# HazyResearch/hyena-dna

Measured on NVIDIA H100. Metric: nucleotides/sec through HyenaOperator fwd+bwd at L=1M d=256, higher is better.
Workload: dtype f32

## Files before the change

hyena-dna_b200/csrc/k_proj.cu:

```cuda
#include <cstdint>
#include <cstring>

#include "../../include/hyena_b200.h"
#include "launch.h"
#include "proj_gemm.cuh"

namespace hy {

static_assert(FN_GELU_TANH == HYENA_B200_GELU_TANH && FN_GELU_ERF == HYENA_B200_GELU_ERF, "activation codes of the C ABI");

size_t proj_wimg_bytes(int N, int K) {
  const int NT = 128;
  return pg::wimg_floats(N, K, NT) * sizeof(float);
}

typedef CUresult (*EncodeTiledFn)(CUtensorMap*, CUtensorMapDataType, cuuint32_t, void*, const cuuint64_t*, const cuuint64_t*,
                                  const cuuint32_t*, const cuuint32_t*, CUtensorMapInterleave, CUtensorMapSwizzle,
                                  CUtensorMapL2promotion, CUtensorMapFloatOOBfill);
static EncodeTiledFn encode_tiled() {
  static EncodeTiledFn fn = [] {
    void* p = nullptr;
    cudaDriverEntryPointQueryResult q;
    if (cudaGetDriverEntryPoint("cuTensorMapEncodeTiled", &p, cudaEnableDefault, &q) != cudaSuccess ||
        q != cudaDriverEntryPointSuccess)
      p = nullptr;
    return reinterpret_cast<EncodeTiledFn>(p);
  }();
  return fn;
}

static bool make_tmap(CUtensorMap* m, const float* base, unsigned long long rows, unsigned long long cols, unsigned box_cols,
                      unsigned box_rows, bool swizzle128) {
  EncodeTiledFn f = encode_tiled();
  if (!f) return false;
  cuuint64_t dims[2] = {cols, rows};
  cuuint64_t strides[1] = {cols * sizeof(float)};
  cuuint32_t box[2] = {box_cols, box_rows};
  cuuint32_t estr[2] = {1, 1};
  return f(m, CU_TENSOR_MAP_DATA_TYPE_FLOAT32, 2, const_cast<float*>(base), dims, strides, box, estr,
           CU_TENSOR_MAP_INTERLEAVE_NONE, swizzle128 ? CU_TENSOR_MAP_SWIZZLE_128B : CU_TENSOR_MAP_SWIZZLE_NONE,
           CU_TENSOR_MAP_L2_PROMOTION_L2_256B, CU_TENSOR_MAP_FLOAT_OOB_FILL_NONE) == CUDA_SUCCESS;
}

static bool make_tmap3(CUtensorMap* m, const float* base, unsigned long long d0, unsigned long long d1, unsigned long long d2,
                       unsigned b0, unsigned b1) {
  EncodeTiledFn f = encode_tiled();
  if (!f) return false;
  cuuint64_t dims[3] = {d0, d1, d2};
  cuuint64_t strides[2] = {d0 * sizeof(float), d0 * d1 * sizeof(float)};
  cuuint32_t box[3] = {b0, b1, 1};
  cuuint32_t estr[3] = {1, 1, 1};
  return f(m, CU_TENSOR_MAP_DATA_TYPE_FLOAT32, 3, const_cast<float*>(base), dims, strides, box, estr,
           CU_TENSOR_MAP_INTERLEAVE_NONE, CU_TENSOR_MAP_SWIZZLE_NONE, CU_TENSOR_MAP_L2_PROMOTION_L2_256B,
           CU_TENSOR_MAP_FLOAT_OOB_FILL_NONE) == CUDA_SUCCESS;
}

template <int NT, int ACT, int OUT, int FN = FN_NONE>
static cudaError_t go(pg::Args a, int sms, cudaStream_t s, int kind = K_PROJ_GEMM) {
  auto kern = pg::proj_gemm_kernel<NT, ACT, OUT, FN>;
  CUtensorMap tmap;
  memset(&tmap, 0, sizeof(tmap));
  if (a.vec) {
    const bool ok = (ACT == pg::ACT_ROW)
        ? make_tmap(&tmap, a.act, (unsigned long long)a.B * a.L, (unsigned long long)a.K, 32, 128, true)
        : make_tmap(&tmap, a.act, (unsigned long long)a.B * a.K, (unsigned long long)a.L, 132, 32, false);
    if (!ok) a.vec = 0;
  }
  const size_t smem = pg::Cfg<NT>::SMEM + (a.fir ? (size_t)a.K * 12 : 0);
  if (smem > 227 * 1024) return cudaErrorInvalidValue;
  cudaError_t e = cudaFuncSetAttribute(kern, cudaFuncAttributeMaxDynamicSharedMemorySize, (int)smem);
  if (e != cudaSuccess) return e;
  const long long ntiles = (long long)a.B * a.mtiles_per_b * a.ntiles_n;
  const int grid = (int)(ntiles < sms ? ntiles : sms);
  prof_begin(kind, s);
  kern<<<grid, pg::kThreads, smem, s>>>(a, tmap);
  prof_end(kind, s);
  return cudaGetLastError();
}

template <int NT>
static cudaError_t by_layout(const pg::Args& a, int act_layout, int out_layout, int sms, cudaStream_t s) {
  if (act_layout == pg::ACT_ROW && out_layout == pg::OUT_CH) return go<NT, pg::ACT_ROW, pg::OUT_CH>(a, sms, s);
  if (act_layout == pg::ACT_ROW && out_layout == pg::OUT_ROW) return go<NT, pg::ACT_ROW, pg::OUT_ROW>(a, sms, s);
  if (act_layout == pg::ACT_CH && out_layout == pg::OUT_CH) return go<NT, pg::ACT_CH, pg::OUT_CH>(a, sms, s);
  if (act_layout == pg::ACT_CH && out_layout == pg::OUT_ROW) return go<NT, pg::ACT_CH, pg::OUT_ROW>(a, sms, s);
  return cudaErrorInvalidValue;
}

cudaError_t launch_proj_gemm(const float* act, int act_layout, const float* W, int ldw, int w_transposed, const float* bias,
                             const float* fir, float* out, int out_layout, int B, int L, int K, int N, int l0, int ln,
                             float* wimg, cudaStream_t s, int fn, const float* aux) {
  const int NT = 128;
  int dev = 0, sms = 132;
  cudaGetDevice(&dev);
  cudaDeviceGetAttribute(&sms, cudaDevAttrMultiProcessorCount, dev);
  const size_t total = pg::wimg_floats(N, K, NT);
  int pblocks = (int)((total + 255) / 256);
  if (pblocks > 4 * sms) pblocks = 4 * sms;
  prof_begin(K_PROJ_PREP, s);
  pg::proj_prep_kernel<<<pblocks, 256, 0, s>>>(W, ldw, w_transposed, N, K, NT, wimg);
  prof_end(K_PROJ_PREP, s);
  cudaError_t e = cudaGetLastError();
  if (e != cudaSuccess) return e;
  pg::Args a;
  a.act = act; a.wimg = wimg; a.out = out; a.bias = bias; a.fir = fir; a.aux = aux;
  a.B = B; a.L = L; a.K = K; a.N = N; a.l0 = l0; a.ln = ln;
  if (act_layout == pg::ACT_ROW) a.vec = (K % 4 == 0);
  else a.vec = (L % 4 == 0) && (l0 % 4 == 0);
  a.kchunks = (K + pg::kKC - 1) / pg::kKC;
  a.ntiles_n = (N + NT - 1) / NT;
  a.mtiles_per_b = (ln + 127) / 128;
  if (fn == FN_NONE) return by_layout<128>(a, act_layout, out_layout, sms, s);
  if (act_layout == pg::ACT_CH && out_layout == pg::OUT_ROW) {
    if (fn == FN_GELU_TANH) return go<128, pg::ACT_CH, pg::OUT_ROW, FN_GELU_TANH>(a, sms, s, K_PROJ_GEMM_GELU);
    if (fn == FN_GELU_ERF) return go<128, pg::ACT_CH, pg::OUT_ROW, FN_GELU_ERF>(a, sms, s, K_PROJ_GEMM_GELU);
  }
  if (act_layout == pg::ACT_ROW && out_layout == pg::OUT_CH) {
    if (fn == FN_GELU_TANH) return go<128, pg::ACT_ROW, pg::OUT_CH, FN_GELU_TANH>(a, sms, s, K_PROJ_GEMM_DGELU);
    if (fn == FN_GELU_ERF) return go<128, pg::ACT_ROW, pg::OUT_CH, FN_GELU_ERF>(a, sms, s, K_PROJ_GEMM_DGELU);
  }
  return cudaErrorInvalidValue;
}


void proj_wgrad_plan(int M, int N, int sms, int* mtiles, int* ntiles, int* splits) {
  *mtiles = (M + 127) / 128;
  *ntiles = (N + 127) / 128;
  int s = sms / (*mtiles * *ntiles);
  *splits = s < 1 ? 1 : s;
}

size_t proj_wgrad_scratch_bytes(int M, int N) {
  int dev = 0, sms = 132, mt, nt, sp;
  cudaGetDevice(&dev);
  cudaDeviceGetAttribute(&sms, cudaDevAttrMultiProcessorCount, dev);
  proj_wgrad_plan(M, N, sms, &mt, &nt, &sp);
  return (size_t)sp * M * N * sizeof(float);
}

cudaError_t launch_proj_wgrad(const float* X, const float* Y, const float* fir, float* dW, int transposed_out, float beta,
                              int B, int L, int M, int N, float* part, cudaStream_t s, int fn) {
  int dev = 0, sms = 132;
  cudaGetDevice(&dev);
  cudaDeviceGetAttribute(&sms, cudaDevAttrMultiProcessorCount, dev);
  wg::Args a;
  a.X = X; a.Y = Y; a.fir = fir; a.part = part; a.zero = 0; a.B = B; a.L = L; a.M = M; a.N = N;
  a.chunks_per_b = (L + 31) / 32;
  proj_wgrad_plan(M, N, sms, &a.mtiles, &a.ntiles, &a.splits);
  const long long total_chunks = (long long)B * a.chunks_per_b;
  if (a.splits > total_chunks) a.splits = (int)total_chunks;
  a.vec = (L % 4 == 0) && (N % 4 == 0) && ((reinterpret_cast<uintptr_t>(X) | reinterpret_cast<uintptr_t>(Y)) & 15u) == 0;
  CUtensorMap tmx, tmy;
  memset(&tmx, 0, sizeof(tmx)); memset(&tmy, 0, sizeof(tmy));
  if (a.vec) {
    const bool ok = make_tmap3(&tmx, X, (unsigned long long)L, (unsigned long long)M, (unsigned long long)B, 36, 128) &&
                    make_tmap3(&tmy, Y, (unsigned long long)N, (unsigned long long)L, (unsigned long long)B, 128, 32);
    if (!ok) a.vec = 0;
  }
  auto kern = fn == FN_GELU_TANH ? wg::wgrad_kernel<FN_GELU_TANH>
            : fn == FN_GELU_ERF  ? wg::wgrad_kernel<FN_GELU_ERF> : wg::wgrad_kernel<FN_NONE>;
  if (fn != FN_NONE && (fir || (fn != FN_GELU_TANH && fn != FN_GELU_ERF))) return cudaErrorInvalidValue;
  const int kind = fn == FN_NONE ? K_PROJ_WGRAD : K_PROJ_WGRAD_GELU;
  cudaError_t e = cudaFuncSetAttribute(kern, cudaFuncAttributeMaxDynamicSharedMemorySize, (int)wg::kSmem);
  if (e != cudaSuccess) return e;
  prof_begin(kind, s);
  kern<<<a.mtiles * a.ntiles * a.splits, wg::kThreads, wg::kSmem, s>>>(a, tmx, tmy);
  prof_end(kind, s);
  e = cudaGetLastError();
  if (e != cudaSuccess) return e;
  const size_t total = (size_t)M * N;
  int blocks = (int)((total + 255) / 256);
  if (blocks > 2 * sms) blocks = 2 * sms;
  prof_begin(kind, s);
  wg::wgrad_reduce_kernel<<<blocks, 256, 0, s>>>(part, dW, a.splits, M, N, transposed_out, beta);
  prof_end(kind, s);
  return cudaGetLastError();
}

}
```

hyena-dna_b200/csrc/proj_gemm.cuh:

```cuda
#pragma once
#include <cuda.h>

#include "common.cuh"
#include "tc_prims.cuh"

namespace hy {

enum ActFn { FN_NONE = 0, FN_GELU_TANH = 1, FN_GELU_ERF = 2 };

template <int FN>
__device__ __forceinline__ float act_fn(float x) {
  static_assert(FN == FN_GELU_TANH || FN == FN_GELU_ERF, "GELU variant");
  if constexpr (FN == FN_GELU_TANH) {
    constexpr float kBeta = (float)(M_SQRT2 * M_2_SQRTPI * 0.5), kKappa = 0.044715f;
    const float inner = kBeta * (x + kKappa * (x * x * x));
    return 0.5f * x * (1.f + tanhf(inner));
  } else {
    return x * 0.5f * (1.f + erff(x * (float)M_SQRT1_2));
  }
}

template <int FN>
__device__ __forceinline__ float act_grad(float x) {
  static_assert(FN == FN_GELU_TANH || FN == FN_GELU_ERF, "GELU variant");
  if constexpr (FN == FN_GELU_TANH) {
    constexpr float kBeta = (float)(M_SQRT2 * M_2_SQRTPI * 0.5), kKappa = 0.044715f;
    const float x_sq = x * x;
    const float th = tanhf(kBeta * (x + kKappa * (x_sq * x)));
    const float left = 0.5f * x, right = 1.f + th;
    const float left_derivative = 0.5f * right;
    const float right_derivative = left * (1.f - th * th) * (kBeta * (1.f + 3.f * kKappa * x_sq));
    return left_derivative + right_derivative;
  } else {
    constexpr float kBeta = (float)(M_2_SQRTPI * M_SQRT1_2 * 0.5);
    const float cdf = 0.5f * (1.f + erff(x * (float)M_SQRT1_2));
    const float pdf = expf(-0.5f * x * x) * kBeta;
    return cdf + x * pdf;
  }
}

namespace pg {

constexpr int kKC = 32;
constexpr int kThreads = 288;
constexpr uint32_t kSBO = 1024, kLBO = 128;
constexpr uint32_t kAPitchCh = 132 * 4;
constexpr uint32_t kAStageBytes = 32 * kAPitchCh;

__host__ __device__ constexpr uint32_t img_off(int n, int k) {
  return (uint32_t)((n >> 3) * 1024 + (k >> 2) * 128 + (n & 7) * 16 + (k & 3) * 4);
}

enum ActLayout { ACT_ROW = 0 , ACT_CH = 1  };
enum OutLayout { OUT_CH = 0 , OUT_ROW = 1  };

struct Args {
  const float* act;
  const float* wimg;
  float* out;
  const float* bias;
  const float* fir;
  int B, L, K, N;
  int l0, ln;
  int kchunks;
  int ntiles_n;
  int mtiles_per_b;
  int vec;
  const float* aux;
};

__global__ void proj_prep_kernel(const float* __restrict__ W, int ldw, int transposed, int N, int K, int NT,
                                 float* __restrict__ img) {
  const int kch = (K + kKC - 1) / kKC, ntn = (N + NT - 1) / NT;
  const size_t total = (size_t)ntn * kch * NT * kKC;
  for (size_t i = (size_t)blockIdx.x * blockDim.x + threadIdx.x; i < total; i += (size_t)gridDim.x * blockDim.x) {
    const int kk = (int)(i % kKC);
    const int nn = (int)((i / kKC) % NT);
    const int kc = (int)((i / ((size_t)kKC * NT)) % kch);
    const int nt = (int)(i / ((size_t)kKC * NT * kch));
    const int n = nt * NT + nn, k = kc * kKC + kk;
    float x = 0.f;
    if (n < N && k < K) x = transposed ? W[(size_t)k * ldw + n] : W[(size_t)n * ldw + k];
    float hi, lo;
    tc::split_tf32(x, hi, lo);
    float* base = img + ((size_t)nt * kch + kc) * 2 * NT * kKC;
    base[img_off(nn, kk) / 4] = hi;
    base[(size_t)NT * kKC + img_off(nn, kk) / 4] = lo;
  }
}

__host__ __device__ constexpr size_t wimg_floats(int N, int K, int NT) {
  return (size_t)((N + NT - 1) / NT) * ((K + kKC - 1) / kKC) * 2 * NT * kKC;
}

constexpr uint32_t kSStageBytes = 17408;
static_assert(kSStageBytes >= 32 * kAPitchCh && kSStageBytes >= 128 * 128 && kSStageBytes % 1024 == 0, "staging slot");

template <int NT> struct Cfg {
  static constexpr int STAGES = 4;
  static constexpr uint32_t STAGE_BYTES = 2u * NT * kKC * 4u;
  static constexpr size_t OFF_A = (size_t)STAGES * STAGE_BYTES;
  static constexpr size_t OFF_BAR = OFF_A + (size_t)STAGES * kSStageBytes;
  static constexpr size_t OFF_FIR = OFF_BAR + 256;
  static constexpr size_t SMEM = OFF_FIR;
  static_assert(NT == 128, "one m64n128 accumulator per consumer warpgroup");
};

template <int NT, int ACT, int OUT, int FN = FN_NONE>
__global__ void __launch_bounds__(kThreads, 1) proj_gemm_kernel(const Args a, const __grid_constant__ CUtensorMap tmap) {
  static_assert(FN == FN_NONE || (ACT == ACT_CH && OUT == OUT_ROW) || (ACT == ACT_ROW && OUT == OUT_CH),
                "the GELU transforms exist for the fc2 forward and input-gradient layouts only");
  using C = Cfg<NT>;
  extern __shared__ __align__(1024) unsigned char smem[];
  uint64_t* bars = reinterpret_cast<uint64_t*>(smem + C::OFF_BAR);
  float* fir_s = reinterpret_cast<float*>(smem + C::OFF_FIR);
  const uint32_t sbase = tc::smem_u32(smem);
  const uint32_t bar0 = tc::smem_u32(bars);
  auto FULL = [&](int s) { return bar0 + 8u * s; };
  auto EMPTY = [&](int s) { return bar0 + 8u * (4 + s); };

  const int tid = threadIdx.x, warp = tid >> 5, lane = tid & 31;
  const bool use_fir = (ACT == ACT_CH) && a.fir != nullptr;
  if (use_fir)
    for (int i = tid; i < 3 * a.K; i += kThreads) fir_s[i] = __ldg(a.fir + i);
  if (tid == 0) {
    for (int s = 0; s < 4; ++s) { tc::mbar_init(FULL(s), 1); tc::mbar_init(EMPTY(s), 8); }
  }
  __syncthreads();

  const int mtiles = a.B * a.mtiles_per_b;
  const int ntiles = mtiles * a.ntiles_n;
  const int lend = a.l0 + a.ln;
  auto tile_pos = [&](int tile, int& b, int& lt, int& nt) {
    const int mt = tile / a.ntiles_n;
    nt = tile - mt * a.ntiles_n;
    b = mt / a.mtiles_per_b;
    lt = a.l0 + (mt - b * a.mtiles_per_b) * 128;
  };

  if (warp == 8) {
    if (lane == 0 && a.vec) tc::tma_prefetch_desc(&tmap);
    uint32_t it = 0;
    for (int tile = blockIdx.x; tile < ntiles; tile += gridDim.x) {
      int b, lt, nt;
      tile_pos(tile, b, lt, nt);
      for (int kc = 0; kc < a.kchunks; ++kc, ++it) {
        const int s = (int)(it & 3u);
        const int k0 = kc * kKC;
        tc::mbar_wait_u(EMPTY(s), ((it >> 2) & 1u) ^ 1u);
        const float* wsrc = a.wimg + ((size_t)nt * a.kchunks + kc) * (C::STAGE_BYTES / 4);
        const uint32_t st_u = sbase + (uint32_t)C::OFF_A + (uint32_t)s * kSStageBytes;
        if (a.vec) {
          if (lane == 0) {
            const uint32_t abytes = (ACT == ACT_ROW) ? 128u * 128u : 32u * kAPitchCh;
            tc::mbar_arrive_expect_tx(FULL(s), C::STAGE_BYTES + abytes);
            tc::bulk_g2s(sbase + s * C::STAGE_BYTES, wsrc, C::STAGE_BYTES, FULL(s));
            if constexpr (ACT == ACT_ROW) tc::tma_load_2d(st_u, &tmap, k0, b * a.L + lt, FULL(s));
            else tc::tma_load_2d(st_u, &tmap, lt, b * a.K + k0, FULL(s));
          }
          continue;
        }
        unsigned char* st = smem + C::OFF_A + (size_t)s * kSStageBytes;
        if constexpr (ACT == ACT_ROW) {
#pragma unroll 1
          for (int i = 0; i < 4; ++i) {
            const int r = lane + 32 * i, l = lt + r;
            const float* src = a.act + ((size_t)b * a.L + (l < lend ? l : 0)) * a.K + k0;
#pragma unroll
            for (int c = 0; c < 8; ++c) {
              float4 v;
              v.x = (l < lend && k0 + 4 * c + 0 < a.K) ? __ldg(src + 4 * c + 0) : 0.f;
              v.y = (l < lend && k0 + 4 * c + 1 < a.K) ? __ldg(src + 4 * c + 1) : 0.f;
              v.z = (l < lend && k0 + 4 * c + 2 < a.K) ? __ldg(src + 4 * c + 2) : 0.f;
              v.w = (l < lend && k0 + 4 * c + 3 < a.K) ? __ldg(src + 4 * c + 3) : 0.f;
              *reinterpret_cast<float4*>(st + r * 128 + ((c ^ (r & 7)) << 4)) = v;
            }
          }
        } else {
          const int j = lane;
          const bool kv = k0 + j < a.K;
          const float* src = a.act + ((size_t)b * a.K + (kv ? k0 + j : 0)) * a.L + lt;
          float* dst = reinterpret_cast<float*>(st + j * kAPitchCh);
          for (int e = 0; e < 132; ++e) dst[e] = (kv && lt + e < a.L) ? __ldg(src + e) : 0.f;
        }
        __syncwarp();
        if (lane == 0) {
          tc::mbar_arrive_expect_tx(FULL(s), C::STAGE_BYTES);
          tc::bulk_g2s(sbase + s * C::STAGE_BYTES, wsrc, C::STAGE_BYTES, FULL(s));
        }
      }
    }
    return;
  }

  const int wg = warp >> 2, g = lane >> 2, t = lane & 3;
  const int r0 = 64 * wg + 16 * (warp & 3) + g;
  uint32_t it = 0;
  for (int tile = blockIdx.x; tile < ntiles; tile += gridDim.x) {
    int b, lt, nt;
    tile_pos(tile, b, lt, nt);
    float sum[64], acc[64];
    for (int kc = 0; kc < a.kchunks; ++kc, ++it) {
      const int s = (int)(it & 3u);
      tc::mbar_wait_u(FULL(s), (it >> 2) & 1u);
      const unsigned char* st = smem + C::OFF_A + (size_t)s * kSStageBytes;
      const int k0 = kc * kKC;
      uint32_t ahi[4][4], alo[4][4];
#pragma unroll
      for (int ks = 0; ks < 4; ++ks) {
#pragma unroll
        for (int q = 0; q < 4; ++q) {
          const int row = r0 + ((q & 1) ? 8 : 0), k = 8 * ks + t + ((q & 2) ? 4 : 0);
          float x;
          if constexpr (ACT == ACT_ROW) {
            x = *reinterpret_cast<const float*>(st + row * 128 + (((k >> 2) ^ (row & 7)) << 4) + (k & 3) * 4);
          } else {
            const float* sp = reinterpret_cast<const float*>(st + k * kAPitchCh) + row;
            if constexpr (FN != FN_NONE) {
              x = act_fn<FN>(sp[0]);
            } else if (!use_fir) {
              x = sp[0];
            } else {
              const float* w = fir_s + 3 * (k0 + k < a.K ? k0 + k : 0);
              x = fmaf(w[2], sp[0], fmaf(w[1], sp[1], w[0] * sp[2]));
            }
          }
          float hh, lw;
          tc::split_tf32(x, hh, lw);
          ahi[ks][q] = __float_as_uint(hh); alo[ks][q] = __float_as_uint(lw);
        }
      }
      const uint32_t bhi = sbase + s * C::STAGE_BYTES, blo = bhi + C::STAGE_BYTES / 2;
      tc::wgmma_fence();
      tc::fence_regs(acc);
#pragma unroll
      for (int ks = 0; ks < 4; ++ks) {
        tc::wgmma_rs_n128(acc, alo[ks], tc::make_desc_ls(bhi + ks * 2 * kLBO, kLBO, kSBO), ks ? 1u : 0u);
        tc::wgmma_rs_n128(acc, ahi[ks], tc::make_desc_ls(blo + ks * 2 * kLBO, kLBO, kSBO), 1u);
      }
#pragma unroll
      for (int ks = 0; ks < 4; ++ks)
        tc::wgmma_rs_n128(acc, ahi[ks], tc::make_desc_ls(bhi + ks * 2 * kLBO, kLBO, kSBO), 1u);
      tc::wgmma_commit();
      tc::wgmma_wait<0>();
      tc::fence_regs(acc);
      __syncwarp();
      if (lane == 0) tc::mbar_arrive(EMPTY(s));
      if (kc == 0) {
#pragma unroll
        for (int i = 0; i < 64; ++i) sum[i] = acc[i];
      } else {
#pragma unroll
        for (int i = 0; i < 64; ++i) sum[i] += acc[i];
      }
    }
#pragma unroll
    for (int h = 0; h < 2; ++h) {
      const int l = lt + r0 + 8 * h;
      if (l >= lend) continue;
      float pre[16];
#pragma unroll
      for (int j = 0; j < 16; ++j) {
        if constexpr (OUT == OUT_CH && FN != FN_NONE) {
          if (j % 8 == 0) {
#pragma unroll
            for (int i = 0; i < 16; ++i) {
              const int n = nt * NT + 8 * (j + (i >> 1)) + 2 * t + (i & 1);
              pre[i] = n < a.N ? __ldg(a.aux + ((size_t)b * a.N + n) * a.L + l) : 0.f;
            }
          }
        }
        const int n = nt * NT + 8 * j + 2 * t;
        float v0 = sum[4 * j + 2 * h], v1 = sum[4 * j + 2 * h + 1];
        if constexpr (OUT == OUT_CH && FN != FN_NONE) {
          float* dst = a.out + ((size_t)b * a.N + n) * a.L + l;
          if (n < a.N) dst[0] = v0 * act_grad<FN>(pre[2 * (j % 8)]);
          if (n + 1 < a.N) dst[a.L] = v1 * act_grad<FN>(pre[2 * (j % 8) + 1]);
        } else if constexpr (OUT == OUT_CH) {
          float* dst = a.out + ((size_t)b * a.N + n) * a.L + l;
          if (n < a.N) dst[0] = v0 + (a.bias ? __ldg(a.bias + n) : 0.f);
          if (n + 1 < a.N) dst[a.L] = v1 + (a.bias ? __ldg(a.bias + n + 1) : 0.f);
        } else {
          float* dst = a.out + ((size_t)b * a.L + l) * a.N + n;
          if (a.bias) {
            if (n < a.N) v0 += __ldg(a.bias + n);
            if (n + 1 < a.N) v1 += __ldg(a.bias + n + 1);
          }
          if (n + 1 < a.N && (a.N & 1) == 0) *reinterpret_cast<float2*>(dst) = make_float2(v0, v1);
          else {
            if (n < a.N) dst[0] = v0;
            if (n + 1 < a.N) dst[1] = v1;
          }
        }
      }
    }
  }
}

}

namespace wg {

constexpr int kThreads = 512;
constexpr int kRegConsumer = 184, kRegConvert = 88, kRegProducer = 56;
static_assert(2 * kRegConsumer + kRegConvert + kRegProducer <= 4 * 128, "register file of one CTA");
constexpr int kSeg = 4;
constexpr int kStg = 4;
constexpr uint32_t kYPitch = 128 * 4;
constexpr uint32_t kYStage = 32 * kYPitch;
constexpr uint32_t kXPitch = 36 * 4;
constexpr uint32_t kXStage = 128 * kXPitch;
constexpr uint32_t kImg = 128 * 32 * 4;
constexpr uint32_t kOffY = 0, kOffX = kOffY + kStg * kYStage;
constexpr uint32_t kOffImg = (kOffX + kStg * kXStage + 1023u) & ~1023u;
constexpr uint32_t kOffBar = kOffImg + 2 * 2 * kImg;
constexpr size_t kSmem = kOffBar + 256;
static_assert(kOffImg % 1024 == 0, "operand images must start on a core-matrix group boundary");
static_assert(kYStage % 128 == 0 && kXStage % 128 == 0, "TMA destinations are 128-byte aligned");
static_assert(kSmem <= 227 * 1024, "shared memory budget");

struct Args {
  const float* X;
  const float* Y;
  const float* fir;
  float* part;
  int B, L, M, N;
  int chunks_per_b;
  int mtiles, ntiles, splits;
  int vec;
  unsigned zero;
};

template <int FN = FN_NONE>
__global__ void __launch_bounds__(kThreads, 1) wgrad_kernel(const Args a, const __grid_constant__ CUtensorMap tmapX,
                                                            const __grid_constant__ CUtensorMap tmapY) {
  extern __shared__ __align__(1024) unsigned char smem[];
  uint64_t* bars = reinterpret_cast<uint64_t*>(smem + kOffBar);
  const uint32_t sbase = tc::smem_u32(smem), bar0 = tc::smem_u32(bars);
  auto B_FULL = [&](int s) { return bar0 + 8u * s; };
  auto B_EMPTY = [&](int s) { return bar0 + 8u * (2 + s); };
  auto S_FULL = [&](int j) { return bar0 + 8u * (4 + j); };
  auto Y_EMPTY = [&](int j) { return bar0 + 8u * (8 + j); };
  auto X_EMPTY = [&](int j) { return bar0 + 8u * (12 + j); };
  const int tid = threadIdx.x, warp = tid >> 5, lane = tid & 31;

  if (tid == 0) {
    for (int s = 0; s < 2; ++s) { tc::mbar_init(B_FULL(s), 128); tc::mbar_init(B_EMPTY(s), 8); }
    for (int j = 0; j < kStg; ++j) { tc::mbar_init(S_FULL(j), 1); tc::mbar_init(Y_EMPTY(j), 256); tc::mbar_init(X_EMPTY(j), 128); }
  }
  __syncthreads();

  const int split = blockIdx.x % a.splits;
  const int tile = blockIdx.x / a.splits;
  const int nt = tile / a.mtiles, mt = tile - nt * a.mtiles;
  const int n0 = nt * 128, m0 = mt * 128;
  const int nrows = min(128, a.N - n0);
  const int mcols = min(128, a.M - m0);
  const long long total_chunks = (long long)a.B * a.chunks_per_b;
  const long long c_begin = total_chunks * split / a.splits, c_end = total_chunks * (split + 1) / a.splits;
  const long long nchunks = c_end - c_begin;

  if (warp < 8) {
    tc::setmaxnreg_inc<kRegConsumer>();
    const int wgi = warp >> 2, g = lane >> 2, t = lane & 3;
    const int nl0 = 64 * wgi + 16 * (warp & 3) + g;
    float acc[64], sum[64], yv[4][4];
#pragma unroll
    for (int i = 0; i < 64; ++i) sum[i] = 0.f;
    auto load_y = [&](long long q) {
      const int ss = (int)(q % kStg);
      tc::mbar_wait_u(S_FULL(ss), (uint32_t)(q / kStg) & 1u);
      const unsigned char* st = smem + kOffY + (size_t)ss * kYStage;
      uint32_t dep = 0;
#pragma unroll
      for (int ks = 0; ks < 4; ++ks) {
#pragma unroll
        for (int e = 0; e < 4; ++e) {
          const int nl = nl0 + ((e & 1) ? 8 : 0), k = 8 * ks + t + ((e & 2) ? 4 : 0);
          yv[ks][e] = *reinterpret_cast<const float*>(st + k * kYPitch + nl * 4);
          dep |= __float_as_uint(yv[ks][e]);
        }
      }
      tc::mbar_arrive_after_loads(Y_EMPTY(ss), dep, a.zero);
    };
    if (nchunks > 0) load_y(0);
    for (long long q = 0; q < nchunks; ++q) {
      uint32_t ahi[4][4], alo[4][4];
#pragma unroll
      for (int ks = 0; ks < 4; ++ks) {
#pragma unroll
        for (int e = 0; e < 4; ++e) {
          float h, lw;
          tc::split_tf32(yv[ks][e], h, lw);
          ahi[ks][e] = __float_as_uint(h); alo[ks][e] = __float_as_uint(lw);
        }
      }
      const uint32_t it = (uint32_t)q;
      const int s = it & 1;
      tc::mbar_wait_u(B_FULL(s), (it >> 1) & 1);
      const uint32_t bhi = sbase + kOffImg + s * 2 * kImg, blo = bhi + kImg;
      const uint32_t cont = (it % kSeg) != 0;
      tc::wgmma_fence();
      tc::fence_regs(acc);
#pragma unroll
      for (int ks = 0; ks < 4; ++ks) {
        tc::wgmma_rs_n128(acc, alo[ks], tc::make_desc_ls(bhi + ks * 2 * pg::kLBO, pg::kLBO, pg::kSBO), (cont | ks) ? 1u : 0u);
        tc::wgmma_rs_n128(acc, ahi[ks], tc::make_desc_ls(blo + ks * 2 * pg::kLBO, pg::kLBO, pg::kSBO), 1u);
      }
#pragma unroll
      for (int ks = 0; ks < 4; ++ks)
        tc::wgmma_rs_n128(acc, ahi[ks], tc::make_desc_ls(bhi + ks * 2 * pg::kLBO, pg::kLBO, pg::kSBO), 1u);
      tc::wgmma_commit();
      if (q + 1 < nchunks) load_y(q + 1);
      tc::wgmma_wait<0>();
      tc::fence_regs(acc);
      tc::fence_frags(ahi);
      tc::fence_frags(alo);
      __syncwarp();
      if (lane == 0) tc::mbar_arrive(B_EMPTY(s));
      if (it % kSeg == kSeg - 1 || q + 1 == nchunks) {
#pragma unroll
        for (int i = 0; i < 64; ++i) sum[i] = acc[i] + sum[i];
      }
    }
#pragma unroll
    for (int h = 0; h < 2; ++h) {
      const int nl = nl0 + 8 * h;
      if (nl >= nrows) continue;
      float* dst = a.part + ((size_t)split * a.N + n0 + nl) * a.M + m0;
#pragma unroll
      for (int j = 0; j < 16; ++j) {
        const int ml = 8 * j + 2 * t;
#pragma unroll
        for (int e = 0; e < 2; ++e)
          if (ml + e < mcols) dst[ml + e] = sum[4 * j + 2 * h + e];
      }
    }
  } else if (warp < 12) {
    tc::setmaxnreg_dec<kRegConvert>();
    const int t = tid - 256;
    const bool use_fir = a.fir != nullptr;
    const int rlo = t & 7, kq = (t >> 3) & 7, rhi0 = t >> 6;
    float w[8][3];
    if (use_fir) {
#pragma unroll
      for (int i = 0; i < 8; ++i) {
        const int m = m0 + rlo + 8 * (rhi0 + 2 * i);
#pragma unroll
        for (int j = 0; j < 3; ++j) w[i][j] = (m < a.M) ? __ldg(a.fir + 3 * m + j) : 0.f;
      }
    }
    for (long long q = 0; q < nchunks; ++q) {
      const int ss = (int)(q % kStg);
      tc::mbar_wait_u(S_FULL(ss), (uint32_t)(q / kStg) & 1u);
      const unsigned char* st = smem + kOffX + (size_t)ss * kXStage;
      const uint32_t it = (uint32_t)q;
      const int s = it & 1;
      tc::mbar_wait_u(B_EMPTY(s), ((it >> 1) & 1) ^ 1);
      unsigned char* hi_img = smem + kOffImg + (size_t)s * 2 * kImg;
      unsigned char* lo_img = hi_img + kImg;
#pragma unroll
      for (int i = 0; i < 8; ++i) {
        const int r = rlo + 8 * (rhi0 + 2 * i);
        const float* row = reinterpret_cast<const float*>(st + r * kXPitch) + 4 * kq;
        float4 v = *reinterpret_cast<const float4*>(row);
        if (use_fir) {
          const float2 nx = *reinterpret_cast<const float2*>(row + 4);
          const float x4 = nx.x, x5 = nx.y;
          float4 o;
          o.x = fmaf(w[i][2], v.x, fmaf(w[i][1], v.y, w[i][0] * v.z));
          o.y = fmaf(w[i][2], v.y, fmaf(w[i][1], v.z, w[i][0] * v.w));
          o.z = fmaf(w[i][2], v.z, fmaf(w[i][1], v.w, w[i][0] * x4));
          o.w = fmaf(w[i][2], v.w, fmaf(w[i][1], x4, w[i][0] * x5));
          v = o;
        }
        if constexpr (FN != FN_NONE) {
          v.x = act_fn<FN>(v.x); v.y = act_fn<FN>(v.y); v.z = act_fn<FN>(v.z); v.w = act_fn<FN>(v.w);
        }
        float4 h, lw;
        tc::split_tf32(v.x, h.x, lw.x); tc::split_tf32(v.y, h.y, lw.y);
        tc::split_tf32(v.z, h.z, lw.z); tc::split_tf32(v.w, h.w, lw.w);
        const uint32_t off = pg::img_off(r, 4 * kq);
        *reinterpret_cast<float4*>(hi_img + off) = h;
        *reinterpret_cast<float4*>(lo_img + off) = lw;
      }
      tc::mbar_arrive(X_EMPTY(ss));
      tc::fence_async_smem();
      tc::mbar_arrive(B_FULL(s));
    }
  } else {
    tc::setmaxnreg_dec<kRegProducer>();
    if (warp != 12) return;
    if (lane == 0 && a.vec) { tc::tma_prefetch_desc(&tmapX); tc::tma_prefetch_desc(&tmapY); }
    int sb_ = (int)(c_begin / a.chunks_per_b), sl_ = (int)(c_begin - (long long)sb_ * a.chunks_per_b) * 32;
    for (long long q = 0; q < nchunks; ++q) {
      const int ss = (int)(q % kStg);
      const uint32_t par = ((uint32_t)(q / kStg) & 1u) ^ 1u;
      const int b = sb_, l0 = sl_;
      sl_ += 32;
      if (sl_ >= a.chunks_per_b * 32) { sl_ = 0; ++sb_; }
      tc::mbar_wait_u(Y_EMPTY(ss), par);
      tc::mbar_wait_u(X_EMPTY(ss), par);
      if (a.vec) {
        if (lane == 0) {
          tc::mbar_arrive_expect_tx(S_FULL(ss), kYStage + kXStage);
          tc::tma_load_3d(sbase + kOffY + ss * kYStage, &tmapY, n0, l0, b, S_FULL(ss));
          tc::tma_load_3d(sbase + kOffX + ss * kXStage, &tmapX, l0, m0, b, S_FULL(ss));
        }
      } else {
        float* ys = reinterpret_cast<float*>(smem + kOffY + (size_t)ss * kYStage);
        for (int i = lane; i < 32 * 128; i += 32) {
          const int k = i >> 7, n = i & 127, l = l0 + k;
          ys[i] = (l < a.L && n0 + n < a.N) ? __ldg(a.Y + ((size_t)b * a.L + l) * a.N + n0 + n) : 0.f;
        }
        float* xs = reinterpret_cast<float*>(smem + kOffX + (size_t)ss * kXStage);
        for (int i = lane; i < 128 * 36; i += 32) {
          const int r = i / 36, e = i - r * 36, l = l0 + e;
          xs[i] = (m0 + r < a.M && l < a.L) ? __ldg(a.X + ((size_t)b * a.M + m0 + r) * a.L + l) : 0.f;
        }
        __syncwarp();
        if (lane == 0) tc::mbar_arrive(S_FULL(ss));
      }
    }
  }
}

__global__ void wgrad_reduce_kernel(const float* __restrict__ part, float* __restrict__ dW, int splits, int M, int N,
                                    int transposed, float beta) {
  const size_t total = (size_t)M * N;
  for (size_t i = (size_t)blockIdx.x * blockDim.x + threadIdx.x; i < total; i += (size_t)gridDim.x * blockDim.x) {
    size_t src;
    if (transposed) src = i;
    else { const int m = (int)(i / N), n = (int)(i - (size_t)m * N); src = (size_t)n * M + m; }
    float s = 0.f;
    for (int k = 0; k < splits; ++k) s += part[(size_t)k * total + src];
    dW[i] = (beta != 0.f) ? fmaf(beta, dW[i], s) : s;
  }
}

}
}
```

Before: 15.30 million.

## Software-pipeline A-fragment loads across wgmma and add register rebalancing

Consumer warps now load and TF32-split the next K-chunk's A fragments while the current wgmma batch runs, double-buffering the fragments in registers and flattening the tile/kchunk loop into one pipelined stream. The block grows to 384 threads so setmaxnreg can give the producer warpgroup fewer registers and the consumers more to hold the extra fragment buffers. The producer's row-layout fill is rewritten so each lane loads one k column across rows. This aims to hide shared-memory fragment loads and the split conversion behind tensor-core work, but it adds register pressure and relies on a release-after-loads barrier trick using a runtime zero.

```diff
diff --git a/hyena-dna_b200/csrc/k_proj.cu b/hyena-dna_b200/csrc/k_proj.cu
--- a/hyena-dna_b200/csrc/k_proj.cu
+++ b/hyena-dna_b200/csrc/k_proj.cu
@@ -103,7 +103,7 @@
   cudaError_t e = cudaGetLastError();
   if (e != cudaSuccess) return e;
   pg::Args a;
-  a.act = act; a.wimg = wimg; a.out = out; a.bias = bias; a.fir = fir; a.aux = aux;
+  a.act = act; a.wimg = wimg; a.out = out; a.bias = bias; a.fir = fir; a.aux = aux; a.zero = 0;
   a.B = B; a.L = L; a.K = K; a.N = N; a.l0 = l0; a.ln = ln;
   if (act_layout == pg::ACT_ROW) a.vec = (K % 4 == 0);
   else a.vec = (L % 4 == 0) && (l0 % 4 == 0);
diff --git a/hyena-dna_b200/csrc/proj_gemm.cuh b/hyena-dna_b200/csrc/proj_gemm.cuh
--- a/hyena-dna_b200/csrc/proj_gemm.cuh
+++ b/hyena-dna_b200/csrc/proj_gemm.cuh
@@ -42,7 +42,9 @@
 namespace pg {
 
 constexpr int kKC = 32;
-constexpr int kThreads = 288;
+constexpr int kThreads = 384;
+constexpr int kRegConsumer = 232, kRegProducer = 40;
+static_assert(2 * kRegConsumer + kRegProducer <= 3 * 168, "register file of one CTA");
 constexpr uint32_t kSBO = 1024, kLBO = 128;
 constexpr uint32_t kAPitchCh = 132 * 4;
 constexpr uint32_t kAStageBytes = 32 * kAPitchCh;
@@ -67,6 +69,7 @@
   int mtiles_per_b;
   int vec;
   const float* aux;
+  unsigned zero;
 };
 
 __global__ void proj_prep_kernel(const float* __restrict__ W, int ldw, int transposed, int N, int K, int NT,
@@ -138,7 +141,9 @@
     lt = a.l0 + (mt - b * a.mtiles_per_b) * 128;
   };
 
-  if (warp == 8) {
+  if (warp >= 8) {
+    tc::setmaxnreg_dec<kRegProducer>();
+    if (warp != 8) return;
     if (lane == 0 && a.vec) tc::tma_prefetch_desc(&tmap);
     uint32_t it = 0;
     for (int tile = blockIdx.x; tile < ntiles; tile += gridDim.x) {
@@ -162,19 +167,13 @@
         }
         unsigned char* st = smem + C::OFF_A + (size_t)s * kSStageBytes;
         if constexpr (ACT == ACT_ROW) {
-#pragma unroll 1
-          for (int i = 0; i < 4; ++i) {
-            const int r = lane + 32 * i, l = lt + r;
-            const float* src = a.act + ((size_t)b * a.L + (l < lend ? l : 0)) * a.K + k0;
-#pragma unroll
-            for (int c = 0; c < 8; ++c) {
-              float4 v;
-              v.x = (l < lend && k0 + 4 * c + 0 < a.K) ? __ldg(src + 4 * c + 0) : 0.f;
-              v.y = (l < lend && k0 + 4 * c + 1 < a.K) ? __ldg(src + 4 * c + 1) : 0.f;
-              v.z = (l < lend && k0 + 4 * c + 2 < a.K) ? __ldg(src + 4 * c + 2) : 0.f;
-              v.w = (l < lend && k0 + 4 * c + 3 < a.K) ? __ldg(src + 4 * c + 3) : 0.f;
-              *reinterpret_cast<float4*>(st + r * 128 + ((c ^ (r & 7)) << 4)) = v;
-            }
+          const int k = lane;
+          const bool kv = k0 + k < a.K;
+#pragma unroll 4
+          for (int r = 0; r < 128; ++r) {
+            const int l = lt + r;
+            const float v = (kv && l < lend) ? __ldg(a.act + ((size_t)b * a.L + l) * a.K + k0 + k) : 0.f;
+            *reinterpret_cast<float*>(st + r * 128 + (((k >> 2) ^ (r & 7)) << 4) + (k & 3) * 4) = v;
           }
         } else {
           const int j = lane;
@@ -193,67 +192,55 @@
     return;
   }
 
+  tc::setmaxnreg_inc<kRegConsumer>();
   const int wg = warp >> 2, g = lane >> 2, t = lane & 3;
   const int r0 = 64 * wg + 16 * (warp & 3) + g;
+  const int my_tiles = (int)blockIdx.x < ntiles ? (ntiles - 1 - (int)blockIdx.x) / (int)gridDim.x + 1 : 0;
+  const uint32_t total = (uint32_t)my_tiles * (uint32_t)a.kchunks;
+
+  auto load_frags = [&](uint32_t (&f)[2][4][4], uint32_t q, int kc) {
+    const int s = (int)(q & 3u);
+    tc::mbar_wait_u(FULL(s), (q >> 2) & 1u);
+    const unsigned char* st = smem + C::OFF_A + (size_t)s * kSStageBytes;
+    const int k0 = kc * kKC;
+#pragma unroll
+    for (int ks = 0; ks < 4; ++ks) {
+#pragma unroll
+      for (int e = 0; e < 4; ++e) {
+        const int row = r0 + ((e & 1) ? 8 : 0), k = 8 * ks + t + ((e & 2) ? 4 : 0);
+        float x;
+        if constexpr (ACT == ACT_ROW) {
+          x = *reinterpret_cast<const float*>(st + row * 128 + (((k >> 2) ^ (row & 7)) << 4) + (k & 3) * 4);
+        } else {
+          const float* sp = reinterpret_cast<const float*>(st + k * kAPitchCh) + row;
+          if constexpr (FN != FN_NONE) {
+            x = act_fn<FN>(sp[0]);
+          } else if (!use_fir) {
+            x = sp[0];
+          } else {
+            const float* w = fir_s + 3 * (k0 + k < a.K ? k0 + k : 0);
+            x = fmaf(w[2], sp[0], fmaf(w[1], sp[1], w[0] * sp[2]));
+          }
+        }
+        float hh, lw;
+        tc::split_tf32(x, hh, lw);
+        f[0][ks][e] = __float_as_uint(hh); f[1][ks][e] = __float_as_uint(lw);
+      }
+    }
+  };
+
+  float sum[64], acc[64];
+  uint32_t fa[2][4][4], fb[2][4][4];
   uint32_t it = 0;
-  for (int tile = blockIdx.x; tile < ntiles; tile += gridDim.x) {
-    int b, lt, nt;
-    tile_pos(tile, b, lt, nt);
-    float sum[64], acc[64];
-    for (int kc = 0; kc < a.kchunks; ++kc, ++it) {
-      const int s = (int)(it & 3u);
-      tc::mbar_wait_u(FULL(s), (it >> 2) & 1u);
-      const unsigned char* st = smem + C::OFF_A + (size_t)s * kSStageBytes;
-      const int k0 = kc * kKC;
-      uint32_t ahi[4][4], alo[4][4];
-#pragma unroll
-      for (int ks = 0; ks < 4; ++ks) {
-#pragma unroll
-        for (int q = 0; q < 4; ++q) {
-          const int row = r0 + ((q & 1) ? 8 : 0), k = 8 * ks + t + ((q & 2) ? 4 : 0);
-          float x;
-          if constexpr (ACT == ACT_ROW) {
-            x = *reinterpret_cast<const float*>(st + row * 128 + (((k >> 2) ^ (row & 7)) << 4) + (k & 3) * 4);
-          } else {
-            const float* sp = reinterpret_cast<const float*>(st + k * kAPitchCh) + row;
-            if constexpr (FN != FN_NONE) {
-              x = act_fn<FN>(sp[0]);
-            } else if (!use_fir) {
-              x = sp[0];
-            } else {
-              const float* w = fir_s + 3 * (k0 + k < a.K ? k0 + k : 0);
-              x = fmaf(w[2], sp[0], fmaf(w[1], sp[1], w[0] * sp[2]));
-            }
-          }
-          float hh, lw;
-          tc::split_tf32(x, hh, lw);
-          ahi[ks][q] = __float_as_uint(hh); alo[ks][q] = __float_as_uint(lw);
-        }
-      }
-      const uint32_t bhi = sbase + s * C::STAGE_BYTES, blo = bhi + C::STAGE_BYTES / 2;
-      tc::wgmma_fence();
-      tc::fence_regs(acc);
-#pragma unroll
-      for (int ks = 0; ks < 4; ++ks) {
-        tc::wgmma_rs_n128(acc, alo[ks], tc::make_desc_ls(bhi + ks * 2 * kLBO, kLBO, kSBO), ks ? 1u : 0u);
-        tc::wgmma_rs_n128(acc, ahi[ks], tc::make_desc_ls(blo + ks * 2 * kLBO, kLBO, kSBO), 1u);
-      }
-#pragma unroll
-      for (int ks = 0; ks < 4; ++ks)
-        tc::wgmma_rs_n128(acc, ahi[ks], tc::make_desc_ls(bhi + ks * 2 * kLBO, kLBO, kSBO), 1u);
-      tc::wgmma_commit();
-      tc::wgmma_wait<0>();
-      tc::fence_regs(acc);
-      __syncwarp();
-      if (lane == 0) tc::mbar_arrive(EMPTY(s));
-      if (kc == 0) {
-#pragma unroll
-        for (int i = 0; i < 64; ++i) sum[i] = acc[i];
-      } else {
-#pragma unroll
-        for (int i = 0; i < 64; ++i) sum[i] += acc[i];
-      }
-    }
+  int kc = 0, tile = blockIdx.x, b = 0, nt = 0;
+  if (total > 0) {
+    int lt_;
+    tile_pos(tile, b, lt_, nt);
+    load_frags(fa, 0, 0);
+  }
+
+  auto store_tile = [&]() {
+    const int lt = a.l0 + (tile / a.ntiles_n - b * a.mtiles_per_b) * 128;
 #pragma unroll
     for (int h = 0; h < 2; ++h) {
       const int l = lt + r0 + 8 * h;
@@ -294,6 +281,55 @@
         }
       }
     }
+  };
+
+  auto step = [&](uint32_t (&cur)[2][4][4], uint32_t (&nxt)[2][4][4]) {
+    const int s = (int)(it & 3u);
+    const uint32_t bhi = sbase + s * C::STAGE_BYTES, blo = bhi + C::STAGE_BYTES / 2;
+    tc::wgmma_fence();
+    tc::fence_regs(acc);
+#pragma unroll
+    for (int ks = 0; ks < 4; ++ks) {
+      tc::wgmma_rs_n128(acc, cur[1][ks], tc::make_desc_ls(bhi + ks * 2 * kLBO, kLBO, kSBO), ks ? 1u : 0u);
+      tc::wgmma_rs_n128(acc, cur[0][ks], tc::make_desc_ls(blo + ks * 2 * kLBO, kLBO, kSBO), 1u);
+    }
+#pragma unroll
+    for (int ks = 0; ks < 4; ++ks)
+      tc::wgmma_rs_n128(acc, cur[0][ks], tc::make_desc_ls(bhi + ks * 2 * kLBO, kLBO, kSBO), 1u);
+    tc::wgmma_commit();
+    const int kn = kc + 1 == a.kchunks ? 0 : kc + 1;
+    if (it + 1 < total) load_frags(nxt, it + 1, kn);
+    tc::wgmma_wait<0>();
+    tc::fence_regs(acc);
+    tc::fence_frags(cur[0]);
+    tc::fence_frags(cur[1]);
+    uint32_t dep = 0;
+#pragma unroll
+    for (int ks = 0; ks < 4; ++ks)
+#pragma unroll
+      for (int e = 0; e < 4; ++e) dep |= cur[0][ks][e];
+    __syncwarp();
+    if (lane == 0) tc::mbar_arrive_after_loads(EMPTY(s), dep, a.zero);
+    if (kc == 0) {
+#pragma unroll
+      for (int i = 0; i < 64; ++i) sum[i] = acc[i];
+    } else {
+#pragma unroll
+      for (int i = 0; i < 64; ++i) sum[i] += acc[i];
+    }
+    if (kn == 0) {
+      store_tile();
+      tile += gridDim.x;
+      int lt_;
+      if (tile < ntiles) tile_pos(tile, b, lt_, nt);
+    }
+    kc = kn;
+    ++it;
+  };
+
+  for (uint32_t q = 0; q < total; q += 2) {
+    step(fa, fb);
+    if (q + 1 < total) step(fb, fa);
   }
 }
 
```

Result: faster. 15.70 million (median of 6 runs) (+2.6%).
